# johanDDC/R-TuckER

Measured on AMD Instinct MI355X. Metric: 1-vs-N triples scored/sec, higher is better.
Workload: dtype f32

## Files before the change

### include/rtucker_hip.h

```cpp
#ifndef RTUCKER_HIP_H
#define RTUCKER_HIP_H

#include <stddef.h>
#include <stdint.h>

#ifdef __cplusplus
extern "C" {
#endif

typedef enum rtk_status {
    RTK_OK = 0,
    RTK_ERR_BAD_ARG = -1,
    RTK_ERR_WORKSPACE = -2,
    RTK_ERR_UNSUPPORTED = -3,
    RTK_ERR_LAUNCH = -4
} rtk_status;

typedef enum rtk_dtype {
    RTK_F32 = 0,
    RTK_BF16 = 1
} rtk_dtype;

#define RTK_SCORE_SIGMOID 1u
#define RTK_SCORE_EXACT_F32 2u
#define RTK_SCORE_SIGMOID_FAST 4u
#define RTK_SCORE_OUT_BF16 8u

#define RTK_SCORE_KERNEL_MASK 0x300u
#define RTK_SCORE_KERNEL_CG 0x100u
#define RTK_SCORE_KERNEL_WS 0x200u
#define RTK_SCORE_KERNEL_V3 0x300u

int rtk_score_kernel_f32(int64_t n_local, int c, unsigned flags);
int64_t rtk_score_fifth_group_columns_f32(int64_t n_local, int c, unsigned flags, unsigned char *mask);

int rtk_version(void);
const char *rtk_last_error_string(void);

size_t rtk_workspace_bytes(int dtype, int64_t batch, int64_t n_rel, int a, int b, int c);

int rtk_read_error_flag(void *workspace, void *stream, uint32_t *host_flag_out);

int rtk_query_vectors_f32(const float *core, int a, int b, int c,
                          const float *R, int64_t n_rel,
                          const float *S, int64_t n_sub,
                          const int64_t *rel_idx, const int64_t *sub_idx, int64_t batch,
                          float *v_out, void *q_packed,
                          void *workspace, size_t workspace_bytes, void *stream);

size_t rtk_packed_query_bytes(int dtype, int64_t batch, int c);

int rtk_pack_query_vectors(const float *v, int64_t batch, int c, int dtype, void *q_packed, void *stream);

size_t rtk_relation_tables_bytes(int64_t n_rel, int b, int c);
size_t rtk_relation_tables_workspace_bytes(int dtype, int64_t n_rel, int a, int b, int c);
size_t rtk_from_tables_workspace_bytes(int64_t batch, int64_t n_rel);

int rtk_relation_tables_f32(const float *core, int a, int b, int c, const float *R, int64_t n_rel,
                            float *tables, void *workspace, size_t workspace_bytes, void *stream);
int rtk_relation_tables_bf16(const void *core, int a, int b, int c, const void *R, int64_t n_rel,
                             float *tables, void *workspace, size_t workspace_bytes, void *stream);

int rtk_query_vectors_from_tables_f32(const float *tables, int64_t n_rel, int b, int c,
                                      const float *S, int64_t n_sub,
                                      const int64_t *rel_idx, const int64_t *sub_idx, int64_t batch,
                                      float *v_out, void *q_packed,
                                      void *workspace, size_t workspace_bytes, void *stream);
int rtk_query_vectors_from_tables_bf16(const float *tables, int64_t n_rel, int b, int c,
                                       const void *S, int64_t n_sub,
                                       const int64_t *rel_idx, const int64_t *sub_idx, int64_t batch,
                                       float *v_out, void *q_packed,
                                       void *workspace, size_t workspace_bytes, void *stream);

int rtk_query_vectors_from_tables_part_f32(const float *tables, int64_t n_rel, int b, int c,
                                           const float *S, int64_t n_sub,
                                           const int64_t *rel_idx, const int64_t *sub_idx, int64_t batch,
                                           int part, int n_parts, float *v_out,
                                           void *workspace, size_t workspace_bytes, void *stream);
int rtk_query_vectors_from_tables_part_bf16(const float *tables, int64_t n_rel, int b, int c,
                                            const void *S, int64_t n_sub,
                                            const int64_t *rel_idx, const int64_t *sub_idx, int64_t batch,
                                            int part, int n_parts, float *v_out,
                                            void *workspace, size_t workspace_bytes, void *stream);

int rtk_score_f32(const float *v, int64_t batch, int c,
                  const float *O, int64_t n_local,
                  float *out, int64_t ld_out, unsigned flags, void *stream);
// ... 187 lines not shown
```

### r-tucker_amd/_lib.py

```python
from __future__ import annotations

import ctypes as C
import os

_HERE = os.path.dirname(os.path.abspath(__file__))
LIB_PATH = os.environ.get("R_TUCKER_AMD_LIB") or os.path.join(_HERE, "lib", "librtucker_hip.so")

RTK_OK = 0
RTK_F32, RTK_BF16 = 0, 1
RTK_SCORE_SIGMOID = 1
RTK_SCORE_EXACT_F32 = 2
RTK_SCORE_SIGMOID_FAST = 4
RTK_SCORE_OUT_BF16 = 8
RTK_SCORE_KERNEL_CG, RTK_SCORE_KERNEL_WS, RTK_SCORE_KERNEL_V3 = 0x100, 0x200, 0x300

_p, _i, _i64, _sz, _u = C.c_void_p, C.c_int, C.c_int64, C.c_size_t, C.c_uint

SIGNATURES = {
    "rtk_version": (_i, []),
    "rtk_last_error_string": (C.c_char_p, []),
    "rtk_workspace_bytes": (_sz, [_i, _i64, _i64, _i, _i, _i]),
    "rtk_packed_query_bytes": (_sz, [_i, _i64, _i]),
    "rtk_read_error_flag": (_i, [_p, _p, C.POINTER(C.c_uint32)]),
    "rtk_query_vectors_f32": (_i, [_p, _i, _i, _i, _p, _i64, _p, _i64, _p, _p, _i64, _p, _p, _p, _sz, _p]),
    "rtk_score_f32": (_i, [_p, _i64, _i, _p, _i64, _p, _i64, _u, _p]),
    "rtk_score_packed_f32": (_i, [_p, _i64, _i, _p, _i64, _p, _i64, _u, _p]),
    "rtk_score_kernel_f32": (_i, [_i64, _i, _u]),
    "rtk_score_fifth_group_columns_f32": (_i64, [_i64, _i, _u, _p]),
    "rtk_score_1vN_f32": (_i, [_p, _i, _i, _i, _p, _i64, _p, _i64, _p, _i64, _p, _p, _i64, _p, _i64, _u, _p, _sz, _p]),
    "rtk_query_vectors_bf16": (_i, [_p, _i, _i, _i, _p, _i64, _p, _i64, _p, _p, _i64, _p, _p, _p, _sz, _p]),
    "rtk_score_packed_bf16": (_i, [_p, _i64, _i, _p, _i64, _p, _i64, _u, _p]),
    "rtk_score_1vN_bf16": (_i, [_p, _i, _i, _i, _p, _i64, _p, _i64, _p, _i64, _p, _p, _i64, _p, _i64, _u, _p, _sz, _p]),
    "rtk_gemm_f32": (_i, [_p, _i, _i64, _p, _i, _i64, _p, _i64, _i64, _i64, _i64, _u, _p]),
    "rtk_gemm_f32_splitk_workspace_bytes": (_sz, [_i64, _i64, _i]),
    "rtk_gemm_f32_splitk": (_i, [_p, _i, _i64, _p, _i, _i64, _p, _i64, _i64, _i64, _i64, _i, _p, _sz, _p]),
    "rtk_gemm_sf16_splitk": (_i, [_p, _i, _i64, _p, _p, _i, _i64, _p, _p, _i64, _i64, _i64, _i64, _i, _p, _sz, _p]),
    "rtk_absmax_f32": (_i, [_p, _i64, _i64, _i64, _p, _p]),
    "rtk_query_bwd_workspace_bytes": (_sz, [_i64, _i, _i, _i]),
    "rtk_query_vectors_bwd_f32": (_i, [_p, _i, _i, _i, _p, _i64, _p, _i64, _p, _p, _i64, _p, _p, _p, _p, _p, _sz, _p]),
    "rtk_pack_query_vectors": (_i, [_p, _i64, _i, _i, _p, _p]),
    "rtk_relation_tables_bytes": (_sz, [_i64, _i, _i]),
    "rtk_relation_tables_workspace_bytes": (_sz, [_i, _i64, _i, _i, _i]),
    "rtk_from_tables_workspace_bytes": (_sz, [_i64, _i64]),
    "rtk_relation_tables_f32": (_i, [_p, _i, _i, _i, _p, _i64, _p, _p, _sz, _p]),
    "rtk_relation_tables_bf16": (_i, [_p, _i, _i, _i, _p, _i64, _p, _p, _sz, _p]),
    "rtk_query_vectors_from_tables_f32": (_i, [_p, _i64, _i, _i, _p, _i64, _p, _p, _i64, _p, _p, _p, _sz, _p]),
    "rtk_query_vectors_from_tables_bf16": (_i, [_p, _i64, _i, _i, _p, _i64, _p, _p, _i64, _p, _p, _p, _sz, _p]),
    "rtk_query_vectors_from_tables_part_f32": (_i, [_p, _i64, _i, _i, _p, _i64, _p, _p, _i64, _i, _i, _p, _p, _sz, _p]),
    "rtk_query_vectors_from_tables_part_bf16": (_i, [_p, _i64, _i, _i, _p, _i64, _p, _p, _i64, _i, _i, _p, _p, _sz, _p]),
    "rtk_sigmoid_grad_f32": (_i, [_p, _p, _p, _i64, _p]),
    "rtk_sigmoid_grad_rows_f32": (_i, [_p, _i64, _p, _i64, _p, _i64, _i64, _i64, _p]),
    "rtk_filtered_rank_f32": (_i, [_p, _i64, _i64, _i64, _p, _p, _p, _p, _p, _p, _p]),
    "rtk_bce_rows_f32": (_i, [_p, _i64, _i64, _i64, _p, _p, _p, C.c_float, _p, _p]),
    "rtk_bce_grad_f32": (_i, [_p, _i64, _i64, _i64, _p, _p, _p, C.c_float, _p, C.c_float, _p]),
    "rtk_rank_metrics_f64": (_i, [_p, _p, _i64, _p, _p]),
    "rtk_rank_metrics_scaled_f64": (_i, [_p, _p, _i64, C.c_double, _p, _p]),
    "rtk_score_bce_partials": (_i, []),
    "rtk_score_packed_bce_f32": (_i, [_p, _i64, _i, _p, _i64, _p, _i64, C.c_float, _p, _p]),
    "rtk_bce_patch_pos_f32": (_i, [_p, _i64, _i64, _i64, _p, _p, _p, C.c_float, _p, _p, _i, _p, _p]),
    "rtk_comm_unique_id": (_i, [_p]),
    "rtk_comm_init": (_i, [_i, _i, _p, C.POINTER(_p)]),
    "rtk_allgather_scores": (_i, [_p, _p, _sz, _p]),
    "rtk_comm_destroy": (_i, [_p]),
    "rtk_timer_create": (_i, [C.POINTER(C.c_void_p)]),
    "rtk_timer_arm": (_i, [_p]),
    "rtk_timer_elapsed_ms": (_i, [_p, C.POINTER(C.c_float)]),
    "rtk_timer_destroy": (_i, [_p]),
    "rtk_gram_factor_f64": (_i, [_p, _i64, _i, _i, C.c_double, C.c_double, _p, _p, _p]),
    "rtk_target_scores_f32": (_i, [_p, _i64, _i64, _i64, _i64, _p, _p, _p]),
    "rtk_filtered_rank_partial_f32": (_i, [_p, _i64, _i64, _i64, _i64, _p, _p, _p, _p, _p, _p, _p, _p]),
    "rtk_select_topk_workspace_bytes": (_sz, [_i64, _i64, _i]),
    "rtk_select_topk_f32": (_i, [_p, _i64, _i64, _i64, _i64, _p, _i64, _p, _p, _p, _p, _i, _p, _p, _p, _sz, _p]),
    "rtk_select_topk_bf16": (_i, [_p, _i64, _i64, _i64, _i64, _p, _i64, _p, _p, _p, _p, _i, _p, _p, _p, _sz, _p]),
    "rtk_score_candidates_f32": (_i, [_p, _i64, _i, _p, _i64, _p, _i64, _i64, _p, _i64, _u, _p, _sz, _p]),
    "rtk_score_candidates_bf16": (_i, [_p, _i64, _i, _p, _i64, _p, _i64, _i64, _p, _i64, _u, _p, _sz, _p]),
    "rtk_score_candidates_bwd_workspace_bytes": (_sz, [_i64, _i64, _i64]),
    "rtk_score_candidates_bwd_f32": (_i, [_p, _i64, _p, _i64, _i, _p, _i64, _p, _i64, _i64, _p, _p, _p, _sz, _p]),
    "rtk_score_candidates_bwd_bf16": (_i, [_p, _i64, _p, _i64, _i, _p, _i64, _p, _i64, _i64, _p, _p, _p, _sz, _p]),
    "rtk_score_rank_workspace_bytes": (_sz, [_i, _i64, _i64, _i]),
    "rtk_score_rank_f32": (_i, [_p, _i64, _i, _p, _i64, _p, _p, _p, _p, _u, _p, _p, _p, _sz, _p]),
    "rtk_score_rank_bf16": (_i, [_p, _i64, _i, _p, _i64, _p, _p, _p, _p, _u, _p, _p, _p, _sz, _p]),
# ... 46 lines not shown
```

### r-tucker_amd/csrc/rtk_query.hip

```cpp
#include "rtk_common.h"
#include "rtk_pack.h"

namespace {

__global__ __launch_bounds__(1024) void plan_kernel(const int64_t *__restrict__ rel_idx, int B, int n_rel,
                                                    int32_t *__restrict__ slot_of_rel,
                                                    int32_t *__restrict__ rel_list,
                                                    uint32_t *__restrict__ flags) {
    __shared__ unsigned count;
    const int t = threadIdx.x;
    if (t == 0) count = 0;
    for (int r = t; r < n_rel; r += blockDim.x) slot_of_rel[r] = -1;
    __syncthreads();
    bool bad = false;
    for (int d = t; d < B; d += blockDim.x) {
        const int64_t r = rel_idx[d];
        if (r < 0 || r >= n_rel) bad = true;
        else slot_of_rel[r] = -2;
    }
    if (bad) atomicOr(&flags[0], 1u);
    __syncthreads();
    for (int r = t; r < n_rel; r += blockDim.x) {
        if (slot_of_rel[r] == -2) {
            const unsigned s = atomicAdd(&count, 1u);
// ... 84 lines not shown
            } else {
                int64_t r = d < B ? rel_idx[d] : 0;
                r = r < 0 ? 0 : (r >= n_rel ? n_rel - 1 : r);
                sl[k] = slot_of_rel ? max(slot_of_rel[r], 0) : (int)r;
                hs[k] = (qinfo && d < B) ? sub_idx[d] : 0;
            }
        }
#pragma unroll
        for (int k = 0; k < CH; ++k) {
            const int d = d0 + NT * k;
            if (d >= B) continue;
            const int pos = atomicAdd(&fill[sl[k]], 1);
            order[pos] = d;
            if (qinfo) {
                qinfo[2 * (int64_t)pos] = hs[k];
                qinfo[2 * (int64_t)pos + 1] = (int64_t)(uint32_t)d | ((int64_t)sl[k] << 32);
            }
        }
    }
}

template <int NT>
__device__ void build_groups(const int64_t *__restrict__ rel_idx, int B, int n_rel,
                             const int32_t *__restrict__ slot_of_rel, int n_slots, int QG,
                             int32_t *__restrict__ cnt_g, int32_t *__restrict__ order,
                             int32_t *__restrict__ work, uint32_t *__restrict__ flags,
                             const int64_t *__restrict__ sub_idx, int64_t *__restrict__ qinfo) {
    __shared__ int sc_q[NT], sc_w[NT];
    __shared__ int base_q, base_w;
    __shared__ int cnt_l[2 * GROUPS_LDS_SLOTS];
    if (n_slots <= GROUPS_LDS_SLOTS)
        build_groups_impl<int *, NT>(rel_idx, B, n_rel, slot_of_rel, n_slots, QG, (int *)cnt_l, order, work, flags, sub_idx, qinfo,
                                     sc_q, sc_w, base_q, base_w);
    else
        build_groups_impl<int32_t *, NT>(rel_idx, B, n_rel, slot_of_rel, n_slots, QG, cnt_g, order, work, flags, sub_idx, qinfo,
                                         sc_q, sc_w, base_q, base_w);
}

struct GroupArgs {
    const int64_t *rel_idx;
    const int32_t *slot_of_rel;
    int32_t *cnt, *order, *work;
    uint32_t *flags;
    int B, n_rel, n_slots, QG;
    const int64_t *sub_idx;
    int64_t *qinfo;
};

__global__ __launch_bounds__(1024) void groups_kernel(GroupArgs ga) {
    build_groups<1024>(ga.rel_idx, ga.B, ga.n_rel, ga.slot_of_rel, ga.n_slots, ga.QG, ga.cnt, ga.order, ga.work, ga.flags, ga.sub_idx, ga.qinfo);
}

constexpr int UT = 4;
template <typename T, bool VEC>
__global__ __launch_bounds__(256) void tables_kernel(const T *__restrict__ G, int a, int64_t bc,
                                                     const T *__restrict__ R,
                                                     const int32_t *__restrict__ rel_list, int n_u_max,
                                                     const uint32_t *__restrict__ n_u_dev,
                                                     float *__restrict__ M, GroupArgs ga) {
    __shared__ float Rs[UT * 64];
    const int xb = ga.QG > 0 ? 1 : 0;
    if (xb && blockIdx.x == 0) {
        if (blockIdx.y == 0) build_groups<256>(ga.rel_idx, ga.B, ga.n_rel, ga.slot_of_rel, ga.n_slots, ga.QG, ga.cnt, ga.order, ga.work, ga.flags, ga.sub_idx, ga.qinfo);
        return;
    }
    const int n_u = n_u_dev ? min(n_u_max, (int)*n_u_dev) : n_u_max;
    const int u0 = blockIdx.y * UT;
    if (u0 >= n_u) return;
    const int t = threadIdx.x;
    constexpr int W = VEC ? 4 : 1;
    constexpr int AB = 16;
    const int64_t n = ((int64_t)(blockIdx.x - xb) * 256 + t) * W;
    const bool live = n < bc;
    float g[AB][W];
    auto load_slices = [&](int a0) {
#pragma unroll
        for (int k = 0; k < AB; ++k) {
            if (live && a0 + k < a) {
                if (VEC) {
                    const f32x4 x = rtk_load4(G + (int64_t)(a0 + k) * bc + n);
#pragma unroll
                    for (int j = 0; j < W; ++j) g[k][j] = x[j];
                } else {
                    g[k][0] = rtk_to_f32(G[(int64_t)(a0 + k) * bc + n]);
                }
            }
        }
    };
    load_slices(0);
    for (int i = t; i < UT * a; i += 256) {
        const int u = u0 + i / a, ai = i % a;
        float x = 0.f;
        if (u < n_u) {
            const int rel = rel_list ? rel_list[u] : u;
            x = rtk_to_f32(R[(int64_t)rel * a + ai]);
        }
        Rs[(i / a) * 64 + ai] = x;
    }
    __syncthreads();
    if (!live) return;
    float acc[UT][W];
#pragma unroll
    for (int u = 0; u < UT; ++u)
#pragma unroll
        for (int j = 0; j < W; ++j) acc[u][j] = 0.f;
    for (int a0 = 0; a0 < a; a0 += AB) {
        if (a0 > 0) load_slices(a0);
#pragma unroll
        for (int k = 0; k < AB; ++k) {
            if (a0 + k < a) {
#pragma unroll
                for (int u = 0; u < UT; ++u) {
                    const float rv = Rs[u * 64 + a0 + k];
#pragma unroll
                    for (int j = 0; j < W; ++j) acc[u][j] = fmaf(rv, g[k][j], acc[u][j]);
                }
            }
// ... 308 lines not shown
                        x += acc[q][j];
                        for (int gg = 1; gg < ngroups; ++gg) x += part[(q * PG + gg - 1) * cpad + k];
                        part[q * PG * cpad + k] = x;
                        mx[q] = fmaxf(mx[q], fabsf(x));
                        if (v_out) v_out[(int64_t)qid[q] * c + k] = x;
                    }
                }
            }
        }
    }
    if (!q_packed) return;
    if (sizeof(T) == 2) {
        __syncthreads();
        for (int q = 0; q < nq; ++q) {
            const int d = qid[q];
            unsigned char *tile = q_packed + (int64_t)(d >> 5) * rtk_pack_tile_bytes(ksteps, 1);
            const int row = d & 31;
            if (t == 0) reinterpret_cast<float *>(tile)[row] = 1.0f;
            rtk_bf16 *plane = reinterpret_cast<rtk_bf16 *>(tile + RTK_PACK_HDR);
            const float *rowv = part + q * PG * cpad;
            for (int k = t; k < ksteps * 16; k += 256)
                plane[rtk_pack_offset(ksteps, k, row)] = rtk_f32_to_bf16((k < c) ? rowv[k] : 0.f);
        }
        return;
    }
#pragma unroll
    for (int q = 0; q < QG; ++q) {
#pragma unroll
        for (int o = 32; o > 0; o >>= 1) mx[q] = fmaxf(mx[q], __shfl_xor(mx[q], o));
        if ((t & 63) == 0) red[t >> 6][q] = mx[q];
    }
    __syncthreads();
    for (int q = 0; q < nq; ++q) {
        const float m = fmaxf(fmaxf(red[0][q], red[1][q]), fmaxf(red[2][q], red[3][q]));
        const int sh = rtk_pack_shift(m);
        const float up = ldexpf(1.0f, sh);
        const int d = qid[q];
        unsigned char *tile = q_packed + (int64_t)(d >> 5) * rtk_pack_tile_bytes(ksteps, 2);
        const int row = d & 31;
        if (t == 0) reinterpret_cast<float *>(tile)[row] = ldexpf(1.0f, -sh);
        _Float16 *planes = reinterpret_cast<_Float16 *>(tile + RTK_PACK_HDR);
        const float *rowv = part + q * PG * cpad;
        for (int k = t; k < ksteps * 16; k += 256) {
            const float x = (k < c) ? rowv[k] * up : 0.f;
            const _Float16 hi = (_Float16)x;
            const _Float16 lo = (_Float16)(x - (float)hi);
            const int off = rtk_pack_offset(ksteps, k, row);
            planes[off] = hi;
            planes[off + ksteps * 512] = lo;
        }
    }
}

template <bool BF16>
__global__ __launch_bounds__(256) void pack_rows_kernel(const float *__restrict__ v, int c, int ksteps,
                                                        unsigned char *__restrict__ q_packed) {
    __shared__ float red[4];
    const int t = threadIdx.x;
    const int64_t d = blockIdx.x;
    const float *row = v + d * c;
    unsigned char *tile = q_packed + (d >> 5) * rtk_pack_tile_bytes(ksteps, BF16 ? 1 : 2);
    const int r = (int)(d & 31);
    if (BF16) {
        if (t == 0) reinterpret_cast<float *>(tile)[r] = 1.0f;
        rtk_bf16 *plane = reinterpret_cast<rtk_bf16 *>(tile + RTK_PACK_HDR);
        for (int k = t; k < ksteps * 16; k += 256) plane[rtk_pack_offset(ksteps, k, r)] = rtk_f32_to_bf16((k < c) ? row[k] : 0.f);
        return;
    }
    float mx = 0.f;
    for (int k = t; k < c; k += 256) mx = fmaxf(mx, fabsf(row[k]));
#pragma unroll
    for (int o = 32; o > 0; o >>= 1) mx = fmaxf(mx, __shfl_xor(mx, o));
    if ((t & 63) == 0) red[t >> 6] = mx;
    __syncthreads();
    mx = fmaxf(fmaxf(red[0], red[1]), fmaxf(red[2], red[3]));
    const int sh = rtk_pack_shift(mx);
    const float up = ldexpf(1.0f, sh);
    if (t == 0) reinterpret_cast<float *>(tile)[r] = ldexpf(1.0f, -sh);
    _Float16 *planes = reinterpret_cast<_Float16 *>(tile + RTK_PACK_HDR);
    for (int k = t; k < ksteps * 16; k += 256) {
        const float x = (k < c) ? row[k] * up : 0.f;
        const _Float16 hi = (_Float16)x;
        const _Float16 lo = (_Float16)(x - (float)hi);
        const int off = rtk_pack_offset(ksteps, k, r);
        planes[off] = hi;
        planes[off + ksteps * 512] = lo;
    }
}

__global__ __launch_bounds__(64) void gather_rel_rows_kernel(const float *__restrict__ R, int a, int n_rel,
                                                             const int32_t *__restrict__ rel_list, float *__restrict__ out) {
    const int u = blockIdx.x;
    int rel = rel_list[u];
    rel = rel < 0 ? 0 : (rel >= n_rel ? n_rel - 1 : rel);
    for (int k = threadIdx.x; k < a; k += 64) out[(int64_t)u * a + k] = R[(int64_t)rel * a + k];
}

}

int rtk_gemm_f32_ex(const void *A, int a_kmajor, int64_t lda, const int32_t *a_rows, const void *B,
                    int b_kmajor, int64_t ldb, float *C, int64_t ldc, int64_t M, int64_t N, int64_t K,
                    unsigned flags, const uint32_t *m_dev, int in_bf16, hipStream_t st);


template <typename T>
static int build_tables(const T *core, int a, int b, int c, const T *R, int64_t n_rel, const int32_t *rel_list,
                        int n_u_max, const uint32_t *n_u_dev, float *tables, void *core_t, void *r_packed,
                        const GroupArgs &ga, hipStream_t st) {
    const int64_t bc = (int64_t)b * c;
    constexpr int VA = rtk_vec4_align<T>();
    const unsigned xb = ga.QG > 0 ? 1u : 0u;
    if (a <= 32) {
        const bool vec = (bc % 4 == 0) && ((reinterpret_cast<uintptr_t>(core) & (VA - 1)) == 0) &&
                         ((reinterpret_cast<uintptr_t>(tables) & 15) == 0);
        const int W = vec ? 4 : 1;
        dim3 grid((unsigned)rtk_cdiv(bc, 256 * W) + xb, (unsigned)rtk_cdiv(n_u_max, UT));
        RTK_REQUIRE(grid.y <= 65535, RTK_ERR_UNSUPPORTED, "relation tables: more than %d relations per launch", 65535 * UT);
        if (vec) hipLaunchKernelGGL((tables_kernel<T, true>), grid, dim3(256), 0, st, core, a, bc, R, rel_list, n_u_max, n_u_dev, tables, ga);
        else hipLaunchKernelGGL((tables_kernel<T, false>), grid, dim3(256), 0, st, core, a, bc, R, rel_list, n_u_max, n_u_dev, tables, ga);
    } else if (sizeof(T) == 2 && core_t && r_packed) {
        const int ks_a = (a + 15) / 16;
        dim3 tg((unsigned)rtk_cdiv(bc, 64) + xb, (unsigned)rtk_cdiv(a, 64));
        hipLaunchKernelGGL(transpose_core_kernel, tg, dim3(256), 0, st, (const rtk_bf16 *)core, a, bc, (rtk_bf16 *)core_t, ga);
        const int rows_padded = (int)rtk_cdiv(n_u_max, 32) * 32;
        hipLaunchKernelGGL(pack_rel_rows_kernel, dim3((unsigned)rows_padded), dim3(256), 0, st, (const rtk_bf16 *)R, a,
                           (int)n_rel, rel_list, n_u_max, n_u_dev, (unsigned char *)r_packed, ks_a);
        int rc = rtk_score_packed_bf16(r_packed, n_u_max, a, core_t, bc, tables, bc, 0, (void *)st);
        if (rc != RTK_OK) return rc;
    } else if (sizeof(T) == 4 && r_packed) {
        if (xb) hipLaunchKernelGGL(groups_kernel, dim3(1), dim3(1024), 0, st, ga);
        float *bounds = (float *)r_packed;
        float *rg = (float *)((unsigned char *)r_packed + 256);
        int rc = rtk_absmax_f32((const float *)R, n_rel, a, a, bounds, (void *)st);
        if (rc != RTK_OK) return rc;
        rc = rtk_absmax_f32((const float *)core, a, bc, bc, bounds + 1, (void *)st);
        if (rc != RTK_OK) return rc;
        const float *A = (const float *)R;
        if (rel_list) {
            hipLaunchKernelGGL(gather_rel_rows_kernel, dim3((unsigned)n_u_max), dim3(64), 0, st, (const float *)R, a, (int)n_rel,
                               rel_list, rg);
            A = rg;
        }
        rc = rtk_gemm_sf16_splitk(A, 1, a, bounds, (const float *)core, 0, bc, bounds + 1, tables, bc, n_u_max, bc, a, 1,
                                  nullptr, 0, (void *)st);
        if (rc != RTK_OK) return rc;
    } else {
        if (xb) hipLaunchKernelGGL(groups_kernel, dim3(1), dim3(1024), 0, st, ga);
        int rc = rtk_gemm_f32_ex(R, 1, a, rel_list, core, 0, bc, tables, bc, n_u_max, bc, a, 0, n_u_dev,
                                 sizeof(T) == 2, st);
        if (rc != RTK_OK) return rc;
    }
    return rtk_check_launch("relation tables");
}

struct ContractPlan {
    bool grouped, cvec;
    int QG;
    size_t smem_grouped;
};
static ContractPlan plan_contract(int b, int c, int64_t batch, const float *tables, int64_t n_slots) {
    ContractPlan p;
    p.cvec = (c % 4 == 0) && ((reinterpret_cast<uintptr_t>(tables) & 15) == 0);
    const int cW = p.cvec ? 4 : 1;
    const int ccols = (c + cW - 1) / cW;
    p.QG = batch >= 2048 ? 8 : 4;
    const int ngroups = ccols <= 256 ? 256 / ccols : 1;
    const int pg = ngroups > 1 ? ngroups - 1 : 1;
    p.smem_grouped = ccols <= 256
        ? (size_t)((size_t)p.QG * ((b + 3) & ~3) + (size_t)p.QG * pg * ccols * cW) * sizeof(float) : (size_t)-1;
    p.grouped = batch >= 2048 && p.smem_grouped <= 64 * 1024 - 1024;
    return p;
}

template <typename T>
static int contract_stage(const float *tables, int b, int c, const T *S, int64_t n_sub, const int64_t *rel_idx,
                          const int64_t *sub_idx, int64_t n_rel, int64_t batch, const int32_t *slot_of_rel,
                          int n_slots, const ContractPlan &cp, bool have_groups, const int32_t *grp_work,
                          const int32_t *grp_order, const int64_t *grp_qinfo, uint32_t *flags, float *v_out,
                          void *q_packed, hipStream_t st, int rel_part = 0, int rel_parts = 1) {
    const int ksteps = (c + 15) / 16;
    if (cp.grouped) {
        RTK_REQUIRE(have_groups, RTK_ERR_BAD_ARG, "rtk_query_vectors: grouped contract without groups");
        const unsigned nwg = (unsigned)(batch / cp.QG + (n_slots < batch ? n_slots : batch) + 8);
#define RTK_CG(V_, Q_) hipLaunchKernelGGL((contract_grouped_kernel<T, V_, Q_>), dim3(nwg), dim3(256), cp.smem_grouped, st, tables, b, c, S, n_sub, rel_idx, sub_idx, (int)n_rel, grp_work, grp_order, v_out, (unsigned char *)q_packed, ksteps, flags, rel_part, rel_parts)
        if (cp.cvec) { if (cp.QG == 8) RTK_CG(true, 8); else RTK_CG(true, 4); }
        else { if (cp.QG == 8) RTK_CG(false, 8); else RTK_CG(false, 4); }
#undef RTK_CG
        return rtk_check_launch("rtk_query_vectors");
    }
    const int W = cp.cvec ? 4 : 1;
    const int cols = (c + W - 1) / W;
    const int ngroups = cols >= 256 ? 1 : 256 / cols;
    const size_t smem = (size_t)ngroups * cols * W * sizeof(float);
    RTK_REQUIRE(smem <= 64 * 1024, RTK_ERR_UNSUPPORTED, "rtk_query_vectors: rank too large for the contract kernel (b=%d c=%d)", b, c);
    const int64_t *pq_order = have_groups ? grp_qinfo : nullptr;
    const unsigned pq_grid = (unsigned)(have_groups ? rtk_cdiv(batch, 8) * 8 : batch);
    if (cp.cvec) hipLaunchKernelGGL((contract_kernel<T, true>), dim3(pq_grid), dim3(256), smem, st, tables, b, c, S, n_sub, rel_idx, sub_idx, (int)n_rel, slot_of_rel, v_out, (unsigned char *)q_packed, ksteps, flags, pq_order, (int)batch, rel_part, rel_parts);
    else hipLaunchKernelGGL((contract_kernel<T, false>), dim3(pq_grid), dim3(256), smem, st, tables, b, c, S, n_sub, rel_idx, sub_idx, (int)n_rel, slot_of_rel, v_out, (unsigned char *)q_packed, ksteps, flags, pq_order, (int)batch, rel_part, rel_parts);
    return rtk_check_launch("rtk_query_vectors");
}

template <typename T>
static int query_vectors_impl(const T *core, int a, int b, int c, const T *R, int64_t n_rel, const T *S,
                              int64_t n_sub, const int64_t *rel_idx, const int64_t *sub_idx, int64_t batch,
                              float *v_out, void *q_packed, const RtkWorkspace &ws, hipStream_t st) {
    const bool planned = n_rel > batch;
    const int n_u_max = (int)(planned ? batch : n_rel);
    if (planned) {
        hipLaunchKernelGGL(plan_kernel, dim3(1), dim3(1024), 0, st, rel_idx, (int)batch, (int)n_rel,
                           ws.slot_of_rel, ws.rel_list, ws.flags);
    }
    const ContractPlan cp = plan_contract(b, c, batch, ws.tables, n_u_max);
    const bool groups = cp.grouped || a > 32;
    GroupArgs ga{rel_idx, planned ? ws.slot_of_rel : nullptr, ws.grp_cnt, ws.grp_order, ws.grp_work, ws.flags,
                 (int)batch, (int)n_rel, n_u_max, groups ? cp.QG : 0, sub_idx, cp.grouped ? nullptr : ws.grp_qinfo};
    int rc = build_tables<T>(core, a, b, c, R, n_rel, planned ? ws.rel_list : nullptr, n_u_max,
                             planned ? ws.flags + 1 : nullptr, ws.tables, ws.core_t, ws.r_packed, ga, st);
    if (rc != RTK_OK) return rc;
    return contract_stage<T>(ws.tables, b, c, S, n_sub, rel_idx, sub_idx, n_rel, batch,
                             planned ? ws.slot_of_rel : nullptr, n_u_max, cp, groups, ws.grp_work, ws.grp_order,
                             ws.grp_qinfo, ws.flags, v_out, q_packed, st);
}

template <typename T>
static int relation_tables_impl(const T *core, int a, int b, int c, const T *R, int64_t n_rel, float *tables,
                                void *core_t, void *r_packed, hipStream_t st) {
    GroupArgs ga{};
    return build_tables<T>(core, a, b, c, R, n_rel, nullptr, (int)n_rel, nullptr, tables, core_t, r_packed, ga, st);
}

template <typename T>
static int from_tables_impl(const float *tables, int64_t n_rel, int b, int c, const T *S, int64_t n_sub,
                            const int64_t *rel_idx, const int64_t *sub_idx, int64_t batch, float *v_out,
                            void *q_packed, const RtkWorkspace &ws, hipStream_t st, int rel_part = 0, int rel_parts = 1) {
    const ContractPlan cp = plan_contract(b, c, batch, tables, n_rel);
    if (cp.grouped) {
        GroupArgs ga{rel_idx, nullptr, ws.grp_cnt, ws.grp_order, ws.grp_work, ws.flags,
                     (int)batch, (int)n_rel, (int)n_rel, cp.QG, sub_idx, nullptr};
        hipLaunchKernelGGL(groups_kernel, dim3(1), dim3(1024), 0, st, ga);
    }
    return contract_stage<T>(tables, b, c, S, n_sub, rel_idx, sub_idx, n_rel, batch, nullptr, (int)n_rel, cp, cp.grouped,
                             ws.grp_work, ws.grp_order, ws.grp_qinfo, ws.flags, v_out, q_packed, st, rel_part, rel_parts);
}

int rtk_query_vectors_f32_impl(const float *core, int a, int b, int c, const float *R, int64_t n_rel,
                               const float *S, int64_t n_sub, const int64_t *rel_idx,
                               const int64_t *sub_idx, int64_t batch, float *v_out, void *q_packed,
                               const RtkWorkspace &ws, hipStream_t st) {
    return query_vectors_impl<float>(core, a, b, c, R, n_rel, S, n_sub, rel_idx, sub_idx, batch, v_out, q_packed, ws, st);
}

int rtk_query_vectors_bf16_impl(const void *core, int a, int b, int c, const void *R, int64_t n_rel,
                                const void *S, int64_t n_sub, const int64_t *rel_idx,
                                const int64_t *sub_idx, int64_t batch, float *v_out, void *q_packed,
                                const RtkWorkspace &ws, hipStream_t st) {
    return query_vectors_impl<rtk_bf16>((const rtk_bf16 *)core, a, b, c, (const rtk_bf16 *)R, n_rel,
                                        (const rtk_bf16 *)S, n_sub, rel_idx, sub_idx, batch, v_out, q_packed, ws, st);
}

int rtk_relation_tables_f32_impl(const float *core, int a, int b, int c, const float *R, int64_t n_rel, float *tables,
                                 void *r_scratch, hipStream_t st) {
    return relation_tables_impl<float>(core, a, b, c, R, n_rel, tables, nullptr, r_scratch, st);
}

int rtk_relation_tables_bf16_impl(const void *core, int a, int b, int c, const void *R, int64_t n_rel, float *tables,
                                  void *core_t, void *r_packed, hipStream_t st) {
    return relation_tables_impl<rtk_bf16>((const rtk_bf16 *)core, a, b, c, (const rtk_bf16 *)R, n_rel, tables, core_t,
                                          r_packed, st);
}

int rtk_from_tables_f32_impl(const float *tables, int64_t n_rel, int b, int c, const float *S, int64_t n_sub,
                             const int64_t *rel_idx, const int64_t *sub_idx, int64_t batch, float *v_out,
                             void *q_packed, const RtkWorkspace &ws, hipStream_t st, int rel_part, int rel_parts) {
    return from_tables_impl<float>(tables, n_rel, b, c, S, n_sub, rel_idx, sub_idx, batch, v_out, q_packed, ws, st, rel_part,
                                   rel_parts);
}

int rtk_from_tables_bf16_impl(const float *tables, int64_t n_rel, int b, int c, const void *S, int64_t n_sub,
                              const int64_t *rel_idx, const int64_t *sub_idx, int64_t batch, float *v_out,
                              void *q_packed, const RtkWorkspace &ws, hipStream_t st, int rel_part, int rel_parts) {
    return from_tables_impl<rtk_bf16>(tables, n_rel, b, c, (const rtk_bf16 *)S, n_sub, rel_idx, sub_idx, batch, v_out,
                                      q_packed, ws, st, rel_part, rel_parts);
}

extern "C" int rtk_pack_query_vectors(const float *v, int64_t batch, int c, int dtype, void *q_packed, void *stream) {
    RTK_REQUIRE(v && q_packed, RTK_ERR_BAD_ARG, "rtk_pack_query_vectors: null operand");
    RTK_REQUIRE(batch > 0 && c > 0 && batch < (1ll << 31), RTK_ERR_BAD_ARG, "rtk_pack_query_vectors: bad sizes");
    RTK_REQUIRE(dtype == RTK_F32 || dtype == RTK_BF16, RTK_ERR_BAD_ARG, "rtk_pack_query_vectors: dtype");
    RTK_REQUIRE(c <= 512, RTK_ERR_UNSUPPORTED, "rtk_pack_query_vectors: c=%d > 512 has no packed score kernel", c);
    hipStream_t st = (hipStream_t)stream;
    const int ks = (c + 15) / 16;
    if (dtype == RTK_BF16) hipLaunchKernelGGL(pack_rows_kernel<true>, dim3((unsigned)batch), dim3(256), 0, st, v, c, ks, (unsigned char *)q_packed);
    else hipLaunchKernelGGL(pack_rows_kernel<false>, dim3((unsigned)batch), dim3(256), 0, st, v, c, ks, (unsigned char *)q_packed);
    return rtk_check_launch("rtk_pack_query_vectors");
}
```

### r-tucker_amd/ops.py

```python
from __future__ import annotations

import ctypes as C
import os

import torch

from . import _lib

_workspaces = {}

DEFAULT_SIGMOID = os.environ.get("R_TUCKER_AMD_SIGMOID", "fast")

ROW_ALIGN = max(1, int(os.environ.get("R_TUCKER_AMD_ROW_ALIGN", "32")))
BACKWARD_GEMM = os.environ.get("R_TUCKER_AMD_BWD_GEMM", "split_fp16")
FUSED_BCE = os.environ.get("R_TUCKER_AMD_FUSED_BCE", "1") == "1"


def _row_pitch(N, dtype):
    unit = ROW_ALIGN * (4 // dtype.itemsize) if ROW_ALIGN > 1 else 1
    return -(-N // unit) * unit


def alloc_scores(B, N, device, lead=(), dtype=torch.float32):
    pitch = _row_pitch(N, dtype)
# ... 929 lines not shown
                _lib.check(lib.rtk_sigmoid_grad_f32(grad_out.data_ptr(), out.data_ptr(), dZ.data_ptr(), out.numel(), sp),
                           "rtk_sigmoid_grad_f32")
            else:
                dZ = grad_out
            want_dv = needs[0] or needs[1] or needs[2]
            dv = torch.empty((B, c), dtype=torch.float32, device=dev) if want_dv else None
            gO = torch.empty((N, c), dtype=torch.float32, device=dev) if needs[3] else None
            nws = lib.rtk_score_candidates_bwd_workspace_bytes(B, K, N) if needs[3] else 0
            ws = torch.empty(max(nws, 256), dtype=torch.uint8, device=dev)
            _lib.check(_entry("rtk_score_candidates_bwd", bf16)(
                dZ.data_ptr(), K, v.data_ptr(), B, c, O.data_ptr(), N, cand.data_ptr(), ctx.ld, K,
                dv.data_ptr() if want_dv else None, gO.data_ptr() if needs[3] else None, ws.data_ptr(), ws.numel(), sp),
                "rtk_score_candidates_bwd")
        if want_dv:
            if bf16:
                core, R, S = core.float(), R.float(), S.float()
            g[0], g[1], g[2] = _stage1_backward(core, R, S, h, r, dv, needs)
        g[3] = gO
        if bf16:
            g = [x.to(pdt) if x is not None else None for x in g]
        return tuple(g) + (None,) * 5


def score_candidates(core, R, S, O, subject_idx, relation_idx, candidates, sigmoid=True, sigmoid_mode=None,
                     tables=None):
    needs_grad = torch.is_grad_enabled() and any(
        isinstance(t, torch.Tensor) and t.requires_grad for t in (core, R, S, O))
    if needs_grad:
        return _ScoreCandidates.apply(core, R, S, O, subject_idx, relation_idx, candidates, sigmoid, sigmoid_mode)
    op = _Operands(core, R, S, O, subject_idx, relation_idx)
    cand, ld, K = _candidates("candidates", candidates, op.B, op.dev)
    flags = _score_flags(sigmoid, sigmoid_mode, torch.float32, op.bf16)
    return _candidate_forward(op, cand, ld, K, flags, tables, want_v=False)[0]


def score_triples(core, R, S, O, subject_idx, relation_idx, object_idx, sigmoid=True, sigmoid_mode=None, tables=None):
    dev = core.device if isinstance(core, torch.Tensor) else None
    t = _idx("object_idx", object_idx, dev) if dev is not None and dev.type == "cuda" else object_idx
    if not isinstance(t, torch.Tensor):
        t = torch.as_tensor(t)
    return score_candidates(core, R, S, O, subject_idx, relation_idx, t.reshape(-1, 1), sigmoid=sigmoid,
                            sigmoid_mode=sigmoid_mode, tables=tables).view(-1)


def cg_fifth_group_columns(N, c, flags=0):
    import numpy as np
    mask = np.zeros(N, dtype=np.uint8)
    n = _lib.load().rtk_score_fifth_group_columns_f32(N, c, flags, mask.ctypes.data)
    if n < 0:
        _lib.check(n, "rtk_score_fifth_group_columns_f32")
    return mask.view(bool)


def check_device_errors(device=None):
    dev = torch.device("cuda", torch.cuda.current_device()) if device is None else torch.device(device)
    bad = None
    for (di, sp), ws in list(_workspaces.items()):
        if di != dev.index:
            continue
        try:
            _check_now(ws, sp)
        except IndexError as e:
            bad = e
    if bad is not None:
        raise bad
```

Measured before the change: 11.42 million.

## Add shared-relation contract kernel that self-groups queries and reuses relation tables

```diff
diff --git a/include/rtucker_hip.h b/include/rtucker_hip.h
--- a/include/rtucker_hip.h
+++ b/include/rtucker_hip.h
@@ -33,6 +33,12 @@
 
 int rtk_score_kernel_f32(int64_t n_local, int c, unsigned flags);
 int64_t rtk_score_fifth_group_columns_f32(int64_t n_local, int c, unsigned flags, unsigned char *mask);
+
+#define RTK_CONTRACT_KERNEL_PER_QUERY 1
+#define RTK_CONTRACT_KERNEL_GROUPED 2
+#define RTK_CONTRACT_KERNEL_SHARED 3
+int rtk_contract_plan(int64_t batch, int64_t n_rel, int b, int c, int from_tables, int *qg, int *rows_in_flight,
+                      int64_t *workgroups);
 
 int rtk_version(void);
 const char *rtk_last_error_string(void);
diff --git a/r-tucker_amd/_lib.py b/r-tucker_amd/_lib.py
--- a/r-tucker_amd/_lib.py
+++ b/r-tucker_amd/_lib.py
@@ -14,6 +14,8 @@
 RTK_SCORE_OUT_BF16 = 8
 RTK_SCORE_KERNEL_CG, RTK_SCORE_KERNEL_WS, RTK_SCORE_KERNEL_V3 = 0x100, 0x200, 0x300
 
+RTK_CONTRACT_KERNEL_PER_QUERY, RTK_CONTRACT_KERNEL_GROUPED, RTK_CONTRACT_KERNEL_SHARED = 1, 2, 3
+
 _p, _i, _i64, _sz, _u = C.c_void_p, C.c_int, C.c_int64, C.c_size_t, C.c_uint
 
 SIGNATURES = {
@@ -27,6 +29,7 @@
     "rtk_score_packed_f32": (_i, [_p, _i64, _i, _p, _i64, _p, _i64, _u, _p]),
     "rtk_score_kernel_f32": (_i, [_i64, _i, _u]),
     "rtk_score_fifth_group_columns_f32": (_i64, [_i64, _i, _u, _p]),
+    "rtk_contract_plan": (_i, [_i64, _i64, _i, _i, _i, C.POINTER(_i), C.POINTER(_i), C.POINTER(_i64)]),
     "rtk_score_1vN_f32": (_i, [_p, _i, _i, _i, _p, _i64, _p, _i64, _p, _i64, _p, _p, _i64, _p, _i64, _u, _p, _sz, _p]),
     "rtk_query_vectors_bf16": (_i, [_p, _i, _i, _i, _p, _i64, _p, _i64, _p, _p, _i64, _p, _p, _p, _sz, _p]),
     "rtk_score_packed_bf16": (_i, [_p, _i64, _i, _p, _i64, _p, _i64, _u, _p]),
diff --git a/r-tucker_amd/csrc/rtk_query.hip b/r-tucker_amd/csrc/rtk_query.hip
--- a/r-tucker_amd/csrc/rtk_query.hip
+++ b/r-tucker_amd/csrc/rtk_query.hip
@@ -160,17 +160,19 @@
 }
 
 constexpr int UT = 4;
-template <typename T, bool VEC>
+template <typename T, bool VEC, bool GROUPS>
 __global__ __launch_bounds__(256) void tables_kernel(const T *__restrict__ G, int a, int64_t bc,
                                                      const T *__restrict__ R,
                                                      const int32_t *__restrict__ rel_list, int n_u_max,
                                                      const uint32_t *__restrict__ n_u_dev,
                                                      float *__restrict__ M, GroupArgs ga) {
     __shared__ float Rs[UT * 64];
-    const int xb = ga.QG > 0 ? 1 : 0;
-    if (xb && blockIdx.x == 0) {
-        if (blockIdx.y == 0) build_groups<256>(ga.rel_idx, ga.B, ga.n_rel, ga.slot_of_rel, ga.n_slots, ga.QG, ga.cnt, ga.order, ga.work, ga.flags, ga.sub_idx, ga.qinfo);
-        return;
+    constexpr int xb = GROUPS ? 1 : 0;
+    if constexpr (GROUPS) {
+        if (blockIdx.x == 0) {
+            if (blockIdx.y == 0) build_groups<256>(ga.rel_idx, ga.B, ga.n_rel, ga.slot_of_rel, ga.n_slots, ga.QG, ga.cnt, ga.order, ga.work, ga.flags, ga.sub_idx, ga.qinfo);
+            return;
+        }
     }
     const int n_u = n_u_dev ? min(n_u_max, (int)*n_u_dev) : n_u_max;
     const int u0 = blockIdx.y * UT;
@@ -585,6 +587,227 @@
     }
 }
 
+constexpr int SH_MAX_REL = 512;
+constexpr int SH_MAX_B = 2048;
+
+template <int QG>
+__device__ __forceinline__ int sh_locate(const int *hist, int n_rel, int item, int &R, int &chunk) {
+    const int lane = threadIdx.x & 63;
+    int base = 0;
+    for (int s0 = 0; s0 < n_rel; s0 += 64) {
+        const int s = s0 + lane;
+        const int nw = s < n_rel ? (hist[s] + QG - 1) / QG : 0;
+        int incl = nw;
+#pragma unroll
+        for (int o = 1; o < 64; o <<= 1) {
+            const int u = __shfl_up(incl, o);
+            if (lane >= o) incl += u;
+        }
+        const int excl = base + incl - nw;
+        const unsigned long long hit = __ballot(item >= excl && item < excl + nw);
+        if (hit) {
+            const int l = __ffsll(hit) - 1;
+            R = s0 + l;
+            chunk = item - __shfl(excl, l);
+        }
+        base += __shfl(incl, 63);
+    }
+    return base;
+}
+
+template <typename T, bool VEC, int QG, int LB>
+__global__ __launch_bounds__(256) void contract_shared_kernel(const float *__restrict__ M, int b, int c,
+                                                              const T *__restrict__ S, int64_t n_sub,
+                                                              const int64_t *__restrict__ rel_idx,
+                                                              const int64_t *__restrict__ sub_idx, int n_rel,
+                                                              float *__restrict__ v_out,
+                                                              unsigned char *__restrict__ q_packed, int ksteps,
+                                                              uint32_t *__restrict__ flags, int B,
+                                                              int rel_part, int rel_parts) {
+    extern __shared__ __attribute__((aligned(16))) float smem[];
+    float *part = smem;
+    __shared__ int hist[SH_MAX_REL];
+    __shared__ int seg_cnt[SH_MAX_B / 64];
+    __shared__ int qid[QG];
+    __shared__ int64_t qh[QG];
+    __shared__ float red[4][QG];
+    constexpr int W = VEC ? 4 : 1;
+    constexpr int KMAX = SH_MAX_B / 256;
+    const int t = threadIdx.x, lane = t & 63, wave = t >> 6;
+
+    int64_t rr[KMAX], hh[KMAX];
+#pragma unroll
+    for (int k = 0; k < KMAX; ++k) {
+        const int d = k * 256 + t;
+        rr[k] = d < B ? rel_idx[d] : -1;
+        hh[k] = d < B ? sub_idx[d] : 0;
+    }
+    for (int s = t; s < n_rel; s += 256) hist[s] = 0;
+    __syncthreads();
+    int rl[KMAX];
+    unsigned badbits = 0;
+#pragma unroll
+    for (int k = 0; k < KMAX; ++k) {
+        rl[k] = -1;
+        if (k * 256 + t < B) {
+            int64_t r = rr[k];
+            if (hh[k] < 0 || hh[k] >= n_sub) { badbits |= 1u << k; hh[k] = 0; }
+            if (r < 0 || r >= n_rel) { badbits |= 1u << k; r = 0; }
+            if (rel_parts <= 1 || (int)r % rel_parts == rel_part) {
+                rl[k] = (int)r;
+                atomicAdd(&hist[rl[k]], 1);
+            }
+        }
+    }
+    __syncthreads();
+
+    int R = 0, chunk = 0;
+    const int n_work = sh_locate<QG>(hist, n_rel, -1, R, chunk);
+    const int n8 = (n_work + 7) / 8;
+    const int item = (blockIdx.x & 7) * n8 + (blockIdx.x >> 3);
+    if ((int)(blockIdx.x >> 3) >= n8 || item >= n_work) return;
+    sh_locate<QG>(hist, n_rel, item, R, chunk);
+    const int nq = min(QG, hist[R] - chunk * QG);
+    const float *Mq = M + (int64_t)R * b * c;
+
+    unsigned long long mem[KMAX];
+#pragma unroll
+    for (int k = 0; k < KMAX; ++k) {
+        mem[k] = 0;
+        if (k * 256 < B) {
+            mem[k] = __ballot(rl[k] == R);
+            if (lane == 0) seg_cnt[k * 4 + wave] = __popcll(mem[k]);
+        }
+    }
+    __syncthreads();
+    {
+        const int nseg = 4 * ((B + 255) / 256);
+        const int n = lane < nseg ? seg_cnt[lane & (SH_MAX_B / 64 - 1)] : 0;
+        int incl = n;
+#pragma unroll
+        for (int o = 1; o < SH_MAX_B / 64; o <<= 1) {
+            const int u = __shfl_up(incl, o);
+            if (lane >= o) incl += u;
+        }
+        const int excl = incl - n;
+#pragma unroll
+        for (int k = 0; k < KMAX; ++k) {
+            if (k * 256 < B) {
+                const int before = __shfl(excl, k * 4 + wave);
+                const int rank = before + __popcll(mem[k] & ((1ull << lane) - 1ull)) - chunk * QG;
+                if (rl[k] == R && rank >= 0 && rank < QG) {
+                    qid[rank] = k * 256 + t;
+                    qh[rank] = hh[k];
+                    if (badbits >> k & 1u) atomicOr(&flags[0], 1u);
+                }
+            }
+        }
+    }
+    __syncthreads();
+
+    const int cols = (c + W - 1) / W;
+    const int cpad = cols * W;
+    const int ngroups = 256 / cols;
+    const T *Sh[QG];
+#pragma unroll
+    for (int q = 0; q < QG; ++q) Sh[q] = S + qh[q < nq ? q : 0] * b;
+    const int g = t / cols, col = t % cols;
+    float acc[QG][W];
+#pragma unroll
+    for (int q = 0; q < QG; ++q)
+#pragma unroll
+        for (int j = 0; j < W; ++j) acc[q][j] = 0.f;
+    if (g < ngroups) {
+        for (int b0 = g; b0 < b; b0 += ngroups * LB) {
+            float x[LB][W], sx[QG][LB];
+#pragma unroll
+            for (int k = 0; k < LB; ++k) {
+                const int bi = b0 + k * ngroups;
+                if (bi < b) {
+#pragma unroll
+                    for (int q = 0; q < QG; ++q) sx[q][k] = rtk_to_f32(Sh[q][bi]);
+                    if (VEC) {
+                        const f32x4 y = *reinterpret_cast<const f32x4 *>(Mq + (int64_t)bi * c + col * 4);
+#pragma unroll
+                        for (int j = 0; j < W; ++j) x[k][j] = y[j];
+                    } else {
+                        x[k][0] = Mq[(int64_t)bi * c + col];
+                    }
+                }
+            }
+#pragma unroll
+            for (int k = 0; k < LB; ++k) {
+                const int bi = b0 + k * ngroups;
+                if (bi < b) {
+#pragma unroll
+                    for (int q = 0; q < QG; ++q)
+#pragma unroll
+                        for (int j = 0; j < W; ++j) acc[q][j] = fmaf(sx[q][k], x[k][j], acc[q][j]);
+                }
+            }
+        }
+#pragma unroll
+        for (int q = 0; q < QG; ++q)
+#pragma unroll
+            for (int j = 0; j < W; ++j) part[(q * ngroups + g) * cpad + col * W + j] = acc[q][j];
+    }
+    __syncthreads();
+    float mx[QG];
+#pragma unroll
+    for (int q = 0; q < QG; ++q) {
+        mx[q] = 0.f;
+        if (q < nq) {
+            float *row = part + q * ngroups * cpad;
+            for (int k = t; k < c; k += 256) {
+                float x = 0.f;
+                for (int gg = 0; gg < ngroups; ++gg) x += row[gg * cpad + k];
+                row[k] = x;
+                mx[q] = fmaxf(mx[q], fabsf(x));
+                if (v_out) v_out[(int64_t)qid[q] * c + k] = x;
+            }
+        }
+    }
+    if (!q_packed) return;
+    if (sizeof(T) == 2) {
+        for (int q = 0; q < nq; ++q) {
+            const int d = qid[q];
+            unsigned char *tile = q_packed + (int64_t)(d >> 5) * rtk_pack_tile_bytes(ksteps, 1);
+            const int row = d & 31;
+            if (t == 0) reinterpret_cast<float *>(tile)[row] = 1.0f;
+            rtk_bf16 *plane = reinterpret_cast<rtk_bf16 *>(tile + RTK_PACK_HDR);
+            const float *rowv = part + q * ngroups * cpad;
+            for (int k = t; k < ksteps * 16; k += 256) plane[rtk_pack_offset(ksteps, k, row)] = rtk_f32_to_bf16((k < c) ? rowv[k] : 0.f);
+        }
+        return;
+    }
+#pragma unroll
+    for (int q = 0; q < QG; ++q) {
+#pragma unroll
+        for (int o = 32; o > 0; o >>= 1) mx[q] = fmaxf(mx[q], __shfl_xor(mx[q], o));
+        if (lane == 0) red[wave][q] = mx[q];
+    }
+    __syncthreads();
+    for (int q = 0; q < nq; ++q) {
+        const float m = fmaxf(fmaxf(red[0][q], red[1][q]), fmaxf(red[2][q], red[3][q]));
+        const int sh = rtk_pack_shift(m);
+        const float up = ldexpf(1.0f, sh);
+        const int d = qid[q];
+        unsigned char *tile = q_packed + (int64_t)(d >> 5) * rtk_pack_tile_bytes(ksteps, 2);
+        const int row = d & 31;
+        if (t == 0) reinterpret_cast<float *>(tile)[row] = ldexpf(1.0f, -sh);
+        _Float16 *planes = reinterpret_cast<_Float16 *>(tile + RTK_PACK_HDR);
+        const float *rowv = part + q * ngroups * cpad;
+        for (int k = t; k < ksteps * 16; k += 256) {
+            const float x = (k < c) ? rowv[k] * up : 0.f;
+            const _Float16 hi = (_Float16)x;
+            const _Float16 lo = (_Float16)(x - (float)hi);
+            const int off = rtk_pack_offset(ksteps, k, row);
+            planes[off] = hi;
+            planes[off + ksteps * 512] = lo;
+        }
+    }
+}
+
 template <bool BF16>
 __global__ __launch_bounds__(256) void pack_rows_kernel(const float *__restrict__ v, int c, int ksteps,
                                                         unsigned char *__restrict__ q_packed) {
@@ -649,8 +872,10 @@
         const int W = vec ? 4 : 1;
         dim3 grid((unsigned)rtk_cdiv(bc, 256 * W) + xb, (unsigned)rtk_cdiv(n_u_max, UT));
         RTK_REQUIRE(grid.y <= 65535, RTK_ERR_UNSUPPORTED, "relation tables: more than %d relations per launch", 65535 * UT);
-        if (vec) hipLaunchKernelGGL((tables_kernel<T, true>), grid, dim3(256), 0, st, core, a, bc, R, rel_list, n_u_max, n_u_dev, tables, ga);
-        else hipLaunchKernelGGL((tables_kernel<T, false>), grid, dim3(256), 0, st, core, a, bc, R, rel_list, n_u_max, n_u_dev, tables, ga);
+#define RTK_TB(V_, G_) hipLaunchKernelGGL((tables_kernel<T, V_, G_>), grid, dim3(256), 0, st, core, a, bc, R, rel_list, n_u_max, n_u_dev, tables, ga)
+        if (vec) { if (xb) RTK_TB(true, true); else RTK_TB(true, false); }
+        else { if (xb) RTK_TB(false, true); else RTK_TB(false, false); }
+#undef RTK_TB
     } else if (sizeof(T) == 2 && core_t && r_packed) {
         const int ks_a = (a + 15) / 16;
         dim3 tg((unsigned)rtk_cdiv(bc, 64) + xb, (unsigned)rtk_cdiv(a, 64));
@@ -686,14 +911,28 @@
     return rtk_check_launch("relation tables");
 }
 
+#ifndef RTK_SHARED_QG
+#define RTK_SHARED_QG 2
+#endif
+#ifndef RTK_SHARED_LB
+#define RTK_SHARED_LB 8
+#endif
+#ifndef RTK_SHARED_MIN_RATIO
+#define RTK_SHARED_MIN_RATIO 8
+#endif
+
 struct ContractPlan {
     bool grouped, cvec;
+    bool shared;
     int QG;
     size_t smem_grouped;
+    int sh_QG, sh_LB;
+    unsigned sh_grid;
+    size_t sh_smem;
 };
-static ContractPlan plan_contract(int b, int c, int64_t batch, const float *tables, int64_t n_slots) {
+static ContractPlan plan_contract(int b, int c, int64_t batch, bool tables_aligned, int64_t n_slots, bool slot_is_rel) {
     ContractPlan p;
-    p.cvec = (c % 4 == 0) && ((reinterpret_cast<uintptr_t>(tables) & 15) == 0);
+    p.cvec = (c % 4 == 0) && tables_aligned;
     const int cW = p.cvec ? 4 : 1;
     const int ccols = (c + cW - 1) / cW;
     p.QG = batch >= 2048 ? 8 : 4;
@@ -702,8 +941,19 @@
     p.smem_grouped = ccols <= 256
         ? (size_t)((size_t)p.QG * ((b + 3) & ~3) + (size_t)p.QG * pg * ccols * cW) * sizeof(float) : (size_t)-1;
     p.grouped = batch >= 2048 && p.smem_grouped <= 64 * 1024 - 1024;
+    p.sh_QG = RTK_SHARED_QG;
+    p.sh_LB = RTK_SHARED_LB;
+    p.sh_grid = 0;
+    p.sh_smem = 0;
+    p.shared = false;
+    if (slot_is_rel && batch < SH_MAX_B && n_slots <= SH_MAX_REL && ccols <= 256) {
+        p.sh_grid = (unsigned)((batch / p.sh_QG + (n_slots < batch ? n_slots : batch) + 7) / 8 * 8);
+        p.sh_smem = (size_t)p.sh_QG * ngroups * ccols * cW * sizeof(float);
+        p.shared = batch >= (int64_t)RTK_SHARED_MIN_RATIO * n_slots;
+    }
     return p;
 }
+static bool tables_aligned16(const float *tables) { return (reinterpret_cast<uintptr_t>(tables) & 15) == 0; }
 
 template <typename T>
 static int contract_stage(const float *tables, int b, int c, const T *S, int64_t n_sub, const int64_t *rel_idx,
@@ -712,6 +962,12 @@
                           const int32_t *grp_order, const int64_t *grp_qinfo, uint32_t *flags, float *v_out,
                           void *q_packed, hipStream_t st, int rel_part = 0, int rel_parts = 1) {
     const int ksteps = (c + 15) / 16;
+    if (cp.shared) {
+#define RTK_CS(V_) hipLaunchKernelGGL((contract_shared_kernel<T, V_, RTK_SHARED_QG, RTK_SHARED_LB>), dim3(cp.sh_grid), dim3(256), cp.sh_smem, st, tables, b, c, S, n_sub, rel_idx, sub_idx, (int)n_rel, v_out, (unsigned char *)q_packed, ksteps, flags, (int)batch, rel_part, rel_parts)
+        if (cp.cvec) RTK_CS(true); else RTK_CS(false);
+#undef RTK_CS
+        return rtk_check_launch("rtk_query_vectors");
+    }
     if (cp.grouped) {
         RTK_REQUIRE(have_groups, RTK_ERR_BAD_ARG, "rtk_query_vectors: grouped contract without groups");
         const unsigned nwg = (unsigned)(batch / cp.QG + (n_slots < batch ? n_slots : batch) + 8);
@@ -743,8 +999,8 @@
         hipLaunchKernelGGL(plan_kernel, dim3(1), dim3(1024), 0, st, rel_idx, (int)batch, (int)n_rel,
                            ws.slot_of_rel, ws.rel_list, ws.flags);
     }
-    const ContractPlan cp = plan_contract(b, c, batch, ws.tables, n_u_max);
-    const bool groups = cp.grouped || a > 32;
+    const ContractPlan cp = plan_contract(b, c, batch, tables_aligned16(ws.tables), n_u_max, !planned);
+    const bool groups = cp.grouped || (a > 32 && !cp.shared);
     GroupArgs ga{rel_idx, planned ? ws.slot_of_rel : nullptr, ws.grp_cnt, ws.grp_order, ws.grp_work, ws.flags,
                  (int)batch, (int)n_rel, n_u_max, groups ? cp.QG : 0, sub_idx, cp.grouped ? nullptr : ws.grp_qinfo};
     int rc = build_tables<T>(core, a, b, c, R, n_rel, planned ? ws.rel_list : nullptr, n_u_max,
@@ -766,7 +1022,7 @@
 static int from_tables_impl(const float *tables, int64_t n_rel, int b, int c, const T *S, int64_t n_sub,
                             const int64_t *rel_idx, const int64_t *sub_idx, int64_t batch, float *v_out,
                             void *q_packed, const RtkWorkspace &ws, hipStream_t st, int rel_part = 0, int rel_parts = 1) {
-    const ContractPlan cp = plan_contract(b, c, batch, tables, n_rel);
+    const ContractPlan cp = plan_contract(b, c, batch, tables_aligned16(tables), n_rel, true);
     if (cp.grouped) {
         GroupArgs ga{rel_idx, nullptr, ws.grp_cnt, ws.grp_order, ws.grp_work, ws.flags,
                      (int)batch, (int)n_rel, (int)n_rel, cp.QG, sub_idx, nullptr};
@@ -814,6 +1070,21 @@
                               void *q_packed, const RtkWorkspace &ws, hipStream_t st, int rel_part, int rel_parts) {
     return from_tables_impl<rtk_bf16>(tables, n_rel, b, c, (const rtk_bf16 *)S, n_sub, rel_idx, sub_idx, batch, v_out,
                                       q_packed, ws, st, rel_part, rel_parts);
+}
+
+extern "C" int rtk_contract_plan(int64_t batch, int64_t n_rel, int b, int c, int from_tables, int *qg, int *rows_in_flight,
+                                 int64_t *workgroups) {
+    RTK_REQUIRE(batch > 0 && batch < (1ll << 31) && n_rel > 0 && b > 0 && c > 0, RTK_ERR_BAD_ARG,
+                "rtk_contract_plan: bad sizes (batch=%lld n_rel=%lld b=%d c=%d)", (long long)batch, (long long)n_rel, b, c);
+    const bool slot_is_rel = from_tables || n_rel <= batch;
+    const ContractPlan p = plan_contract(b, c, batch, true, slot_is_rel ? n_rel : batch, slot_is_rel);
+    if (qg) *qg = p.shared ? p.sh_QG : (p.grouped ? p.QG : 1);
+    if (rows_in_flight) *rows_in_flight = p.shared ? p.sh_LB : (p.grouped ? (p.QG <= 4 ? 20 : 8) : 8);
+    if (workgroups) {
+        const int64_t n_slots = slot_is_rel ? n_rel : batch;
+        *workgroups = p.shared ? (int64_t)p.sh_grid : (p.grouped ? batch / p.QG + (n_slots < batch ? n_slots : batch) + 8 : batch);
+    }
+    return p.shared ? RTK_CONTRACT_KERNEL_SHARED : (p.grouped ? RTK_CONTRACT_KERNEL_GROUPED : RTK_CONTRACT_KERNEL_PER_QUERY);
 }
 
 extern "C" int rtk_pack_query_vectors(const float *v, int64_t batch, int c, int dtype, void *q_packed, void *stream) {
diff --git a/r-tucker_amd/ops.py b/r-tucker_amd/ops.py
--- a/r-tucker_amd/ops.py
+++ b/r-tucker_amd/ops.py
@@ -1005,6 +1005,19 @@
     return mask.view(bool)
 
 
+def contract_plan(batch, n_rel, b, c, from_tables=False):
+    import ctypes as C
+    qg, rows, wgs = C.c_int(), C.c_int(), C.c_int64()
+    k = _lib.load().rtk_contract_plan(batch, n_rel, b, c, int(from_tables), C.byref(qg), C.byref(rows), C.byref(wgs))
+    if k < 0:
+        _lib.check(k, "rtk_contract_plan")
+    return k, qg.value, rows.value, wgs.value
+
+
+def contract_kernel(batch, n_rel, b, c, from_tables=False):
+    return contract_plan(batch, n_rel, b, c, from_tables)[0]
+
+
 def check_device_errors(device=None):
     dev = torch.device("cuda", torch.cuda.current_device()) if device is None else torch.device(device)
     bad = None
```

Result: slower. 11.25 million (-1.5%).
